# orgTestCodacy11KRepos110MB/repo-8852-ginkgo

Measured on AMD Instinct MI355X. Metric: CSR SpMV GFLOP/s (fp64, 1M-row 5-pt Poisson per GPU), higher is better.
Workload: dtype f64; 1 GPU; benchmark/spmv: CSR fp64/int32 y=Ax on 1000x1000 5-pt Poisson (n=1e6, nnz=4996000), x=sin(0.01 i); cache_state=cold: rotating over 8 copies (> 256 MiB Infinity Cache), partition=one GPU

## Files before the change

include/gkomi.h:

```cpp
#ifndef GKOMI_H_
#define GKOMI_H_

#include <stddef.h>
#include <stdint.h>

#ifdef __cplusplus
extern "C" {
#endif

typedef void* gkomi_stream_t;

enum {
    GKOMI_SUCCESS = 0,
    GKOMI_EINVAL = -1,
    GKOMI_ENOTSUPPORTED = -2,
    GKOMI_ENOTIMPL = -3,
    GKOMI_EWORKSPACE = -4,
    GKOMI_ECOMM = -5,
    GKOMI_ETRS_OVERRUN = -6
};

#define GKOMI_STATUS_CONVERGED 0x80u
#define GKOMI_STATUS_FINALIZED 0x40u
#define GKOMI_STATUS_ID_MASK 0x3fu
// ... 547 lines not shown
    gkomi_stream_t s, int64_t iterations, int64_t nnz,
    const int32_t* coo_row_idxs, const int32_t* coo_col_idxs,
    const double* coo_vals, const int32_t* l_row_ptrs,
    const int32_t* l_col_idxs, double* l_vals, const int32_t* ut_row_ptrs,
    const int32_t* ut_col_idxs, double* ut_vals);
int gkomi_factorization_initialize_row_ptrs_l_i32(
    gkomi_stream_t s, int64_t n, const int32_t* row_ptrs,
    const int32_t* col_idxs, int32_t* l_row_ptrs, void* workspace,
    size_t workspace_bytes);
int gkomi_factorization_initialize_l_f64_i32(
    gkomi_stream_t s, int64_t n, const int32_t* row_ptrs,
    const int32_t* col_idxs, const double* vals, const int32_t* l_row_ptrs,
    int32_t* l_col_idxs, double* l_vals, int diag_sqrt);
int gkomi_par_ic_init_factor_f64_i32(gkomi_stream_t s, int64_t n,
                                     const int32_t* l_row_ptrs,
                                     const int32_t* l_col_idxs, double* l_vals);
int gkomi_par_ic_compute_factor_f64_i32(gkomi_stream_t s, int64_t iterations,
                                        int64_t l_nnz,
                                        const int32_t* l_row_idxs,
                                        const double* a_lower_vals,
                                        const int32_t* l_row_ptrs,
                                        const int32_t* l_col_idxs,
                                        double* l_vals);
size_t gkomi_ilu_analysis_workspace_bytes(int64_t n);
void gkomi_ilu_tuning(int64_t* host_out);
int gkomi_ilu_analyse_i32(gkomi_stream_t s, int64_t n, const int32_t* row_ptrs,
                          const int32_t* col_idxs, void* workspace,
                          size_t workspace_bytes, int64_t* host_out);
int gkomi_ilu_compute_lu_f64_i32(gkomi_stream_t s, int64_t n,
                                 const int32_t* row_ptrs,
                                 const int32_t* col_idxs, double* vals,
                                 const void* analysis_workspace,
                                 size_t workspace_bytes);
int gkomi_ic_compute_f64_i32(gkomi_stream_t s, int64_t n,
                             const int32_t* row_ptrs, const int32_t* col_idxs,
                             double* vals, const void* analysis_workspace,
                             size_t workspace_bytes);
int gkomi_elimination_forest_host_i32(int64_t n, const int32_t* host_row_ptrs,
                                      const int32_t* host_col_idxs,
                                      int32_t* parents, int32_t* child_ptrs,
                                      int32_t* children, int32_t* postorder,
                                      int32_t* inv_postorder,
                                      int32_t* postorder_parents);
int gkomi_elimination_forest_i32(gkomi_stream_t s, int64_t n,
                                 const int32_t* row_ptrs,
                                 const int32_t* col_idxs, int32_t* parents,
                                 int32_t* child_ptrs, int32_t* children,
                                 int32_t* postorder, int32_t* inv_postorder,
                                 int32_t* postorder_parents);
size_t gkomi_cholesky_symbolic_workspace_bytes(int64_t n, int64_t nnz);
int gkomi_cholesky_symbolic_count_i32(gkomi_stream_t s, int64_t n, int64_t nnz,
                                      const int32_t* row_ptrs,
                                      const int32_t* col_idxs,
                                      const int32_t* inv_postorder,
                                      const int32_t* postorder_parents,
                                      int32_t* row_nnz, void* workspace,
                                      size_t workspace_bytes,
                                      int64_t* host_factor_nnz);
int gkomi_cholesky_symbolic_factorize_i32(
    gkomi_stream_t s, int64_t n, int64_t nnz, const int32_t* row_ptrs,
    const int32_t* col_idxs, const int32_t* postorder,
    const int32_t* inv_postorder, const int32_t* postorder_parents,
    const int32_t* out_row_ptrs, int32_t* out_cols, void* workspace,
    size_t workspace_bytes);
int gkomi_lu_initialize_f64_i32(gkomi_stream_t s, int64_t n,
                                const int32_t* a_row_ptrs,
                                const int32_t* a_col_idxs, const double* a_vals,
                                int64_t factor_nnz, const int32_t* f_row_ptrs,
                                const int32_t* f_col_idxs, double* f_vals,
                                int32_t* diag_idxs, void* workspace,
                                size_t workspace_bytes);
int gkomi_lu_factorize_f64_i32(gkomi_stream_t s, int64_t n,
                               const int32_t* f_row_ptrs,
                               const int32_t* f_col_idxs, double* f_vals,
                               const void* analysis_workspace,
                               size_t workspace_bytes);
int gkomi_lu_symbolic_supported(int has_symbolic, int symmetric_sparsity);

size_t gkomi_matrix_data_workspace_bytes(int64_t nnz);
int gkomi_matrix_data_sort_row_major_f64_i32(gkomi_stream_t s, int64_t nnz,
                                             int32_t* row_idxs,
                                             int32_t* col_idxs, double* values,
                                             void* workspace,
                                             size_t workspace_bytes);
int gkomi_matrix_data_remove_zeros_f64_i32(
    gkomi_stream_t s, int64_t nnz, const int32_t* row_idxs,
    const int32_t* col_idxs, const double* values, int32_t* out_row_idxs,
    int32_t* out_col_idxs, double* out_values, void* workspace,
    size_t workspace_bytes, int64_t* host_nnz);
int gkomi_matrix_data_sum_duplicates_f64_i32(
    gkomi_stream_t s, int64_t nnz, const int32_t* row_idxs,
    const int32_t* col_idxs, const double* values, int32_t* out_row_idxs,
    int32_t* out_col_idxs, double* out_values, void* workspace,
    size_t workspace_bytes, int64_t* host_nnz);

int gkomi_csr_sort_by_column_index_f64_i32(gkomi_stream_t s, int64_t nrows,
                                           const int32_t* row_ptrs,
                                           int32_t* col_idxs, double* vals);
int gkomi_csr_is_sorted_by_column_index_i32(gkomi_stream_t s, int64_t nrows,
                                            const int32_t* row_ptrs,
                                            const int32_t* col_idxs,
                                            void* workspace,
                                            size_t workspace_bytes,
                                            int* host_is_sorted);
size_t gkomi_csr_transpose_workspace_bytes(int64_t ncols);
int gkomi_csr_transpose_f64_i32(gkomi_stream_t s, int64_t nrows, int64_t ncols,
                                int64_t nnz, const int32_t* row_ptrs,
                                const int32_t* col_idxs, const double* vals,
                                int32_t* t_row_ptrs, int32_t* t_col_idxs,
                                double* t_vals, void* workspace,
                                size_t workspace_bytes);

size_t gkomi_csr_spgemm_workspace_bytes(int64_t a_nrows, int64_t b_ncols);
int gkomi_csr_spgemm_f64_i32(
    gkomi_stream_t s, int64_t a_nrows, int64_t a_ncols, int64_t a_nnz,
    const int32_t* a_row_ptrs, const int32_t* a_col_idxs, const double* a_vals,
    int64_t b_nrows, int64_t b_ncols, int64_t b_nnz, const int32_t* b_row_ptrs,
    const int32_t* b_col_idxs, const double* b_vals, const double* alpha,
    const double* beta, int64_t d_nrows, int64_t d_ncols, int64_t d_nnz,
    const int32_t* d_row_ptrs, const int32_t* d_col_idxs, const double* d_vals,
    int32_t* c_row_ptrs, int32_t* c_col_idxs, double* c_vals,
    int64_t* host_c_nnz, void* workspace, size_t workspace_bytes);
int gkomi_csr_spgemm_bins(int64_t out[3]);
size_t gkomi_csr_spgeam_workspace_bytes(int64_t nrows);
int gkomi_csr_spgeam_f64_i32(
    gkomi_stream_t s, int64_t nrows, int64_t ncols, const double* alpha,
    int64_t a_nnz, const int32_t* a_row_ptrs, const int32_t* a_col_idxs,
    const double* a_vals, const double* beta, int64_t b_nrows, int64_t b_ncols,
    int64_t b_nnz, const int32_t* b_row_ptrs, const int32_t* b_col_idxs,
    const double* b_vals, int32_t* c_row_ptrs, int32_t* c_col_idxs,
    double* c_vals, int64_t* host_c_nnz, void* workspace,
    size_t workspace_bytes);

typedef int (*gkomi_apply_fn)(void* ctx, gkomi_stream_t s, const double* in,
                              double* out);
size_t gkomi_cg_workspace_bytes(int64_t n, int64_t nrhs);
size_t gkomi_diag_radix_sort_workspace_bytes(int64_t n, int key_bytes, int pairs);
int gkomi_diag_radix_sort(gkomi_stream_t s, int64_t n, int key_bytes, const void* keys_in,
                          void* keys_out, const uint32_t* vals_in, uint32_t* vals_out,
                          int end_bit, void* workspace, size_t workspace_bytes);
int gkomi_diag_scan_i32(gkomi_stream_t s, int kind, const int32_t* in, int32_t* out,
                        int64_t n, void* workspace, size_t workspace_bytes);
int gkomi_diag_stream_csr_bytes(gkomi_stream_t s, int blocks, int64_t nrows,
                                int64_t nnz, const int32_t* row_ptrs,
                                const int32_t* col_idxs, const double* vals,
                                const double* b, double* c);
int gkomi_diag_poisson3d_7pt_f64_i32(gkomi_stream_t s, int64_t g, int32_t* row_ptrs,
                                     int32_t* col_idxs, double* vals);
int gkomi_diag_poisson3d_7pt_f64_i64(gkomi_stream_t s, int64_t g, int64_t* row_ptrs,
                                     int64_t* col_idxs, double* vals);
int64_t gkomi_diag_csr_evicted_applies(void);
int64_t gkomi_cg_persistent_solves(void);
int gkomi_cg_persistent_enable(int mode);
int64_t gkomi_gmres_meeting_fallbacks(void);
int gkomi_cg_solve_f64_i32(gkomi_stream_t s, int64_t n, int64_t nrhs,
                           int64_t nnz, const int32_t* row_ptrs,
                           const int32_t* col_idxs, const double* vals,
                           int spmv_strategy, int64_t max_row_nnz_hint,
                           gkomi_apply_fn precond, void* precond_ctx,
                           const double* b, double* x, int64_t max_iters,
                           double reduction_factor, int baseline, int mode,
                           int check_every, void* workspace,
                           size_t workspace_bytes, double* host_info);

int gkomi_bicgstab_initialize_f64(gkomi_stream_t s, int64_t n, int64_t nrhs,
    const double* b, int64_t b_stride, double* r, int64_t r_stride, double*
    rr, int64_t rr_stride, double* y, int64_t y_stride, double* s_vec, int64_t
    s_stride, double* t, int64_t t_stride, double* z, int64_t z_stride,
    double* v, int64_t v_stride, double* p, int64_t p_stride, double*
    prev_rho, double* rho, double* alpha, double* beta, double* gamma, double*
    omega, uint8_t* stop_status);
int gkomi_bicgstab_step_1_f64(gkomi_stream_t s, int64_t n, int64_t nrhs, const
    double* r, int64_t r_stride, double* p, int64_t p_stride, const double* v,
    int64_t v_stride, const double* rho, const double* prev_rho, const double*
    alpha, const double* omega, const uint8_t* stop_status);
int gkomi_bicgstab_step_2_f64(gkomi_stream_t s, int64_t n, int64_t nrhs, const
    double* r, int64_t r_stride, double* s_vec, int64_t s_stride, const
    double* v, int64_t v_stride, const double* rho, double* alpha, const
    double* beta, const uint8_t* stop_status);
int gkomi_bicgstab_step_3_f64(gkomi_stream_t s, int64_t n, int64_t nrhs,
    double* x, int64_t x_stride, double* r, int64_t r_stride, const double*
    s_vec, int64_t s_stride, const double* t, int64_t t_stride, const double*
    y, int64_t y_stride, const double* z, int64_t z_stride, const double*
    alpha, const double* beta, const double* gamma, double* omega, const
    uint8_t* stop_status);
int gkomi_bicgstab_finalize_f64(gkomi_stream_t s, int64_t n, int64_t nrhs,
    double* x, int64_t x_stride, const double* y, int64_t y_stride, const
    double* alpha, uint8_t* stop_status);
int gkomi_fcg_initialize_f64(gkomi_stream_t s, int64_t n, int64_t nrhs, const
    double* b, int64_t b_stride, double* r, int64_t r_stride, double* z,
    int64_t z_stride, double* p, int64_t p_stride, double* q, int64_t
    q_stride, double* t, int64_t t_stride, double* prev_rho, double* rho,
    double* rho_t, uint8_t* stop_status);
int gkomi_fcg_step_1_f64(gkomi_stream_t s, int64_t n, int64_t nrhs, double* p,
    int64_t p_stride, const double* z, int64_t z_stride, const double* rho_t,
    const double* prev_rho, const uint8_t* stop_status);
int gkomi_fcg_step_2_f64(gkomi_stream_t s, int64_t n, int64_t nrhs, double* x,
    int64_t x_stride, double* r, int64_t r_stride, double* t, int64_t
    t_stride, const double* p, int64_t p_stride, const double* q, int64_t
    q_stride, const double* beta, const double* rho, const uint8_t*
    stop_status);
int gkomi_cgs_initialize_f64(gkomi_stream_t s, int64_t n, int64_t nrhs, const
    double* b, int64_t b_stride, double* r, int64_t r_stride, double* r_tld,
    int64_t r_tld_stride, double* p, int64_t p_stride, double* q, int64_t
    q_stride, double* u, int64_t u_stride, double* u_hat, int64_t
    u_hat_stride, double* v_hat, int64_t v_hat_stride, double* t, int64_t
    t_stride, double* alpha, double* beta, double* gamma, double* prev_rho,
    double* rho, uint8_t* stop_status);
int gkomi_cgs_step_1_f64(gkomi_stream_t s, int64_t n, int64_t nrhs, const
    double* r, int64_t r_stride, double* u, int64_t u_stride, double* p,
    int64_t p_stride, const double* q, int64_t q_stride, double* beta, const
    double* rho, const double* prev_rho, const uint8_t* stop_status);
int gkomi_cgs_step_2_f64(gkomi_stream_t s, int64_t n, int64_t nrhs, const
    double* u, int64_t u_stride, const double* v_hat, int64_t v_hat_stride,
    double* q, int64_t q_stride, double* t, int64_t t_stride, double* alpha,
    const double* rho, const double* gamma, const uint8_t* stop_status);
int gkomi_cgs_step_3_f64(gkomi_stream_t s, int64_t n, int64_t nrhs, const
    double* t, int64_t t_stride, const double* u_hat, int64_t u_hat_stride,
    double* r, int64_t r_stride, double* x, int64_t x_stride, const double*
    alpha, const uint8_t* stop_status);
size_t gkomi_krylov_workspace_bytes(int64_t n, int64_t nrhs);
int gkomi_bicgstab_solve_f64_i32(gkomi_stream_t s, int64_t n, int64_t nrhs,
    int64_t nnz, const int32_t* row_ptrs, const int32_t* col_idxs, const
    double* vals, int spmv_strategy, int64_t max_row_nnz_hint, gkomi_apply_fn
    precond, void* precond_ctx, const double* b, double* x, int64_t max_iters,
    double reduction_factor, int baseline, int64_t check_every, void* workspace, size_t
    workspace_bytes, double* host_info);
int gkomi_fcg_solve_f64_i32(gkomi_stream_t s, int64_t n, int64_t nrhs, int64_t
    nnz, const int32_t* row_ptrs, const int32_t* col_idxs, const double* vals,
    int spmv_strategy, int64_t max_row_nnz_hint, gkomi_apply_fn precond, void*
    precond_ctx, const double* b, double* x, int64_t max_iters, double
    reduction_factor, int baseline, int64_t check_every, void* workspace, size_t workspace_bytes,
    double* host_info);
int gkomi_cgs_solve_f64_i32(gkomi_stream_t s, int64_t n, int64_t nrhs, int64_t
    nnz, const int32_t* row_ptrs, const int32_t* col_idxs, const double* vals,
    int spmv_strategy, int64_t max_row_nnz_hint, gkomi_apply_fn precond, void*
    precond_ctx, const double* b, double* x, int64_t max_iters, double
    reduction_factor, int baseline, int64_t check_every, void* workspace, size_t workspace_bytes,
    double* host_info);

int gkomi_bicg_initialize_f64(gkomi_stream_t s, int64_t n, int64_t nrhs, const
    double* b, int64_t b_stride, double* r, int64_t r_stride, double* z,
    int64_t z_stride, double* p, int64_t p_stride, double* q, int64_t
    q_stride, double* prev_rho, double* rho, double* r2, int64_t r2_stride,
    double* z2, int64_t z2_stride, double* p2, int64_t p2_stride, double* q2,
    int64_t q2_stride, uint8_t* stop_status);
int gkomi_bicg_step_1_f64(gkomi_stream_t s, int64_t n, int64_t nrhs, double*
    p, int64_t p_stride, const double* z, int64_t z_stride, double* p2,
    int64_t p2_stride, const double* z2, int64_t z2_stride, const double* rho,
    const double* prev_rho, const uint8_t* stop_status);
int gkomi_bicg_step_2_f64(gkomi_stream_t s, int64_t n, int64_t nrhs, double*
    x, int64_t x_stride, double* r, int64_t r_stride, double* r2, int64_t
    r2_stride, const double* p, int64_t p_stride, const double* q, int64_t
    q_stride, const double* q2, int64_t q2_stride, const double* beta, const
    double* rho, const uint8_t* stop_status);
int gkomi_ir_initialize(gkomi_stream_t s, int64_t nrhs, uint8_t* stop_status);
int gkomi_bicg_solve_f64_i32(gkomi_stream_t s, int64_t n, int64_t nrhs,
    int64_t nnz, const int32_t* row_ptrs, const int32_t* col_idxs, const
    double* vals, const int32_t* t_row_ptrs, const int32_t* t_col_idxs, const
    double* t_vals, int spmv_strategy, int64_t max_row_nnz_hint,
    gkomi_apply_fn precond, void* precond_ctx, gkomi_apply_fn precond_t, void*
    precond_t_ctx, const double* b, double* x, int64_t max_iters, double
    reduction_factor, int baseline, int64_t check_every, void* workspace,
    size_t workspace_bytes, double* host_info);
int gkomi_ir_solve_f64_i32(gkomi_stream_t s, int64_t n, int64_t nrhs, int64_t
    nnz, const int32_t* row_ptrs, const int32_t* col_idxs, const double* vals,
    int spmv_strategy, int64_t max_row_nnz_hint, gkomi_apply_fn inner, void*
    inner_ctx, double relaxation_factor, const double* b, double* x, int64_t
    max_iters, double reduction_factor, int baseline, void* workspace, size_t
    workspace_bytes, double* host_info);

int gkomi_partition_build_ranges_from_global_size(int64_t num_parts,
                                                  int64_t global_size,
                                                  int64_t* host_ranges);
int gkomi_partition_build_from_contiguous(int64_t num_parts,
                                          const int64_t* host_ranges,
                                          int64_t* host_range_bounds,
                                          int32_t* host_part_ids);
int gkomi_partition_build_from_mapping(int64_t n, const int32_t* host_mapping,
                                       int64_t* host_range_bounds,
                                       int32_t* host_part_ids,
                                       int64_t* host_num_ranges);
int gkomi_partition_build_starting_indices(const int64_t* host_range_bounds,
                                           const int32_t* host_part_ids,
                                           int64_t num_ranges,
                                           int64_t num_parts,
                                           int32_t* host_starting_indices,
                                           int32_t* host_part_sizes,
                                           int64_t* host_num_empty_parts);
int gkomi_partition_has_ordered_parts(const int32_t* host_part_ids,
                                      int64_t num_ranges, int64_t* host_result);
int gkomi_dist_vector_build_local_f64(gkomi_stream_t s, int64_t nnz,
                                      const int64_t* rows, const int64_t* cols,
                                      const double* vals, const int64_t* range_bounds,
                                      const int32_t* part_ids, const int32_t* starts,
                                      int64_t num_ranges, int32_t local_part,
                                      double* local, int64_t local_stride);
size_t gkomi_dist_build_workspace_bytes(int64_t nnz);
int gkomi_dist_build_local_nonlocal_sizes(
    gkomi_stream_t s, int64_t nnz, const int64_t* rows, const int64_t* cols,
    const int64_t* row_range_bounds, const int32_t* row_part_ids,
    const int32_t* row_starts, int64_t row_num_ranges,
    const int64_t* col_range_bounds, const int32_t* col_part_ids,
    const int32_t* col_starts, int64_t col_num_ranges, int32_t local_part,
    void* workspace, size_t workspace_bytes, int64_t host_sizes[3]);
int gkomi_dist_build_local_nonlocal_fill(
// ... 388 lines not shown
```

repo-8852-ginkgo_amd/csrc/cg_persistent.hpp:

```cpp
#pragma once
#include "cg_fused.hpp"

namespace gkomi {
namespace {

constexpr int pcg_block = 1024;
constexpr int pcg_items = 6;
constexpr int pcg_tile = pcg_block * pcg_items;
constexpr int pcg_max_rows_per_thread = 8;
constexpr int pcg_max_stride = 256;
constexpr int pcg_default_stride = 16;

struct pcg_slot {
    unsigned long long v_bits;
    unsigned long long check;
};

struct pcg_control {
    unsigned int overrun;
    unsigned int pad_[15];
    unsigned long long ticks[8];
    unsigned long long pad2_[16];
};

#ifdef GKOMI_PCG_PROFILE
#define PCG_STAMP(i)                                      \
    do {                                                  \
        const unsigned long long now_ = wall_clock64();   \
        if (blockIdx.x == 0 && threadIdx.x == 0) ctl->ticks[i] += now_ - stamp_; \
        stamp_ = now_;                                    \
    } while (0)
#else
#define PCG_STAMP(i)
#endif

typedef unsigned int pcg_u32x4 __attribute__((ext_vector_type(4)));

__device__ __forceinline__ unsigned long long pcg_key(long long meeting)
{
    return static_cast<unsigned long long>(meeting) * 0x9e3779b97f4a7c15ull;
}

__device__ __forceinline__ void pcg_publish(pcg_slot* slot, double v, long long meeting)
{
    const unsigned long long bits = static_cast<unsigned long long>(__double_as_longlong(v));
    const unsigned long long chk = bits ^ pcg_key(meeting);
    pcg_u32x4 w;
    w.x = static_cast<unsigned int>(bits);
    w.y = static_cast<unsigned int>(bits >> 32);
    w.z = static_cast<unsigned int>(chk);
    w.w = static_cast<unsigned int>(chk >> 32);
    asm volatile("global_store_dwordx4 %0, %1, off sc1" : : "v"(slot), "v"(w) : "memory");
}

__device__ __forceinline__ bool pcg_fetch(const pcg_slot* slot, long long meeting, double* v)
{
    pcg_u32x4 w;
    asm volatile("global_load_dwordx4 %0, %1, off sc1\n\ts_waitcnt vmcnt(0)" : "=v"(w) : "v"(slot) : "memory");
    const unsigned long long bits = (static_cast<unsigned long long>(w.y) << 32) | w.x;
    const unsigned long long chk = (static_cast<unsigned long long>(w.w) << 32) | w.z;
    *v = __longlong_as_double(static_cast<long long>(bits));
    return (bits ^ chk) == pcg_key(meeting);
}

constexpr int pcg_copies = 32;

__device__ __forceinline__ void pcg_sync_lds()
{
    asm volatile("s_waitcnt lgkmcnt(0)\n\ts_barrier" ::: "memory");
}

template <int Block>
__device__ __forceinline__ double pcg_block_sum(double v, double* smem)
{
    v = wave_reduce_sum(v);
    if ((threadIdx.x & 63) == 0) smem[threadIdx.x >> 6] = v;
    pcg_sync_lds();
    double total = 0.0;
#pragma unroll
    for (int w = 0; w < Block / wave_size; ++w) total += smem[w];
    pcg_sync_lds();
    return total;
}

template <int Block>
__device__ __forceinline__ bool pcg_meet(pcg_slot* slots, int stride, int nap, int nwg, long long meeting,
                                         double mine, double* smem, pcg_control* ctl, long long max_polls,
                                         double* total)
{
    constexpr int nwaves = Block / wave_size;
    pcg_slot* bank = slots + (meeting & 1) * static_cast<int64_t>(nwg + pcg_copies) * stride;
    pcg_slot* back = bank + static_cast<int64_t>(nwg) * stride;
#ifdef GKOMI_PCG_PROFILE
    const unsigned long long m0_ = wall_clock64();
#endif
    if (threadIdx.x == 0) pcg_publish(bank + blockIdx.x * stride, mine, meeting);
    bool ok = true;
    auto wait_for = [&](const pcg_slot* slot, double* v) {
        long long polls = 0;
        while (!pcg_fetch(slot, meeting, v)) {
            for (int z = 0; z < nap; ++z) __builtin_amdgcn_s_sleep(1);
            if (++polls > max_polls ||
                ((polls & 255) == 0 &&
                 __hip_atomic_load(&ctl->overrun, __ATOMIC_RELAXED, __HIP_MEMORY_SCOPE_AGENT) != 0)) {
                *v = 0.0;
                return false;
            }
        }
        return true;
    };
    if (threadIdx.x == 0) smem[nwaves] = 1.0;
    pcg_sync_lds();
    double sum = 0.0;
    if (blockIdx.x == 0) {
        double part = 0.0;
        if (static_cast<int>(threadIdx.x) < nwg) ok = wait_for(bank + threadIdx.x * stride, &part);
#ifdef GKOMI_PCG_PROFILE
        if (threadIdx.x == 0) ctl->pad2_[0] += wall_clock64() - m0_;
        if (threadIdx.x == nwg - 1) ctl->pad2_[1] += wall_clock64() - m0_;
#endif
        if (!ok) smem[nwaves] = 0.0;
        part = wave_reduce_sum(part);
        if ((threadIdx.x & 63) == 0) smem[threadIdx.x >> 6] = part;
        pcg_sync_lds();
#pragma unroll
        for (int w = 0; w < nwaves; ++w) sum += smem[w];
        ok = smem[nwaves] != 0.0;
        if (ok && threadIdx.x < pcg_copies) pcg_publish(back + threadIdx.x * stride, sum, meeting);
#ifdef GKOMI_PCG_PROFILE
        if (threadIdx.x == 0) ctl->pad2_[2] += wall_clock64() - m0_;
#endif
    } else {
        if (threadIdx.x == 0) {
            ok = wait_for(back + (blockIdx.x % pcg_copies) * stride, &sum);
#ifdef GKOMI_PCG_PROFILE
            if (blockIdx.x == 101) ctl->pad2_[3] += wall_clock64() - m0_;
            if (blockIdx.x == 101) ctl->pad2_[4] += 1;
#endif
            smem[0] = sum;
            if (!ok) smem[nwaves] = 0.0;
        }
        pcg_sync_lds();
        sum = smem[0];
        ok = smem[nwaves] != 0.0;
    }
    pcg_sync_lds();
    if (!ok) {
        if (threadIdx.x == 0) __hip_atomic_store(&ctl->overrun, 1u, __ATOMIC_RELAXED, __HIP_MEMORY_SCOPE_AGENT);
        return false;
    }
    *total = sum;
    return true;
}

template <int Block, int NV, bool Published = false, typename F>
__device__ __forceinline__ bool pcg_meet_values(pcg_slot* slots, int stride, int nap, int nwg, long long meeting,
                                                double* lsum, double* lred, double* lval, pcg_control* ctl,
                                                long long max_polls, F after_publish)
{
    static_assert(NV <= pcg_default_stride, "a workgroup's values share its slot line");
    static_assert(pcg_copies * NV <= Block, "one thread per copy and value");
    constexpr int nwaves = Block / wave_size;
    const int tid = threadIdx.x;
    pcg_slot* bank = slots + (meeting & 1) * static_cast<int64_t>(nwg + pcg_copies) * stride;
    pcg_slot* back = bank + static_cast<int64_t>(nwg) * stride;
    if (!Published && tid < NV) pcg_publish(bank + blockIdx.x * stride + tid, lsum[tid], meeting);
    after_publish();
    if (!Published) {
        if (tid == 0) lred[nwaves * NV] = 1.0;
        pcg_sync_lds();
    }
    const unsigned long long key = pcg_key(meeting);
    bool ok = true;
    if (blockIdx.x == 0) {
        if (Published) pcg_sync_lds();
        constexpr int U = 5;
        const int npairs = nwg * NV;
        for (int base = 0; base < npairs && ok; base += U * Block) {
            unsigned int pending = 0u;
#pragma unroll
            for (int u = 0; u < U; ++u) {
                if (base + u * Block + tid < npairs) pending |= 1u << u;
            }
            long long polls = 0;
            while (pending != 0u) {
                unsigned long long bits[U], chk[U];
#pragma unroll
                for (int u = 0; u < U; ++u) {
                    if ((pending >> u) & 1u) {
                        const int pr = base + u * Block + tid;
                        const pcg_slot* slot = bank + (pr / NV) * stride + pr % NV;
                        bits[u] = __hip_atomic_load(&slot->v_bits, __ATOMIC_RELAXED, __HIP_MEMORY_SCOPE_AGENT);
                        chk[u] = __hip_atomic_load(&slot->check, __ATOMIC_RELAXED, __HIP_MEMORY_SCOPE_AGENT);
                    }
                }
#pragma unroll
                for (int u = 0; u < U; ++u) {
                    if (((pending >> u) & 1u) && (bits[u] ^ chk[u]) == key) {
                        lval[base + u * Block + tid] = __longlong_as_double(static_cast<long long>(bits[u]));
                        pending &= ~(1u << u);
                    }
                }
                if (pending != 0u) {
                    for (int z = 0; z < nap; ++z) __builtin_amdgcn_s_sleep(1);
                    if (++polls > max_polls ||
                        ((polls & 255) == 0 &&
                         __hip_atomic_load(&ctl->overrun, __ATOMIC_RELAXED, __HIP_MEMORY_SCOPE_AGENT) != 0)) {
                        ok = false;
                        break;
                    }
                }
            }
        }
        if (!ok) lred[nwaves * NV] = 0.0;
        pcg_sync_lds();
        ok = lred[nwaves * NV] != 0.0;
        if (ok) {
            for (int v = tid >> 6; v < NV; v += nwaves) {
                double t = 0.0;
                for (int g = tid & 63; g < nwg; g += wave_size) t += lval[g * NV + v];
                t = wave_reduce_sum(t);
                if ((tid & 63) == 0) lsum[v] = t;
            }
        }
        pcg_sync_lds();
        ok = lred[nwaves * NV] != 0.0;
        if (ok && tid < pcg_copies * NV) pcg_publish(back + (tid / NV) * stride + tid % NV, lsum[tid % NV], meeting);
    } else {
        if (tid < NV) {
            double total = 0.0;
            long long polls = 0;
            while (!pcg_fetch(back + (blockIdx.x % pcg_copies) * stride + tid, meeting, &total)) {
                for (int z = 0; z < nap; ++z) __builtin_amdgcn_s_sleep(1);
                if (++polls > max_polls ||
                    ((polls & 255) == 0 &&
                     __hip_atomic_load(&ctl->overrun, __ATOMIC_RELAXED, __HIP_MEMORY_SCOPE_AGENT) != 0)) {
                    lred[nwaves * NV] = 0.0;
                    total = 0.0;
                    break;
                }
            }
            lsum[tid] = total;
        }
        pcg_sync_lds();
        ok = lred[nwaves * NV] != 0.0;
    }
    pcg_sync_lds();
    if (!ok) {
        if (tid == 0) __hip_atomic_store(&ctl->overrun, 1u, __ATOMIC_RELAXED, __HIP_MEMORY_SCOPE_AGENT);
        return false;
    }
    return true;
}

template <int Block>
__device__ __forceinline__ bool pcg_barrier(pcg_slot* slots, int stride, int nap, int nwg, long long meeting,
                                            double* smem, pcg_control* ctl, long long max_polls)
{
    __builtin_amdgcn_s_waitcnt(0);
    pcg_sync_lds();
    double unused;
    return pcg_meet<Block>(slots, stride, nap, nwg, meeting, 0.0, smem, ctl, max_polls, &unused);
}

template <int R, int K, int Block, bool XL = false>
__global__ __launch_bounds__(Block) void cg_persistent_kernel(
    int n, int chunk, const int32_t* __restrict__ row_ptrs, const int32_t* __restrict__ col_idxs,
    const double* __restrict__ vals, double* __restrict__ x, double* __restrict__ r, double* pbuf0,
    double* pbuf1, pcg_slot* slots, int stride, int nap, pcg_control* ctl, cg_scalars* scal,
    long long max_iters, double goal, long long max_polls, int ell_stored, int64_t ell_stride)
{
    typedef double nt_double2 __attribute__((ext_vector_type(2)));
    typedef int nt_int2 __attribute__((ext_vector_type(2)));
    constexpr int pairs = pcg_items / 2;
    __shared__ __attribute__((aligned(16))) double prod[K > 0 ? 2 : (Block * pcg_items)];
    __shared__ unsigned int lcol[K > 0 ? K * R * Block : 1];
    __shared__ double lx[XL ? R * Block : 1];
    __shared__ double smem[Block / wave_size + 1];
    const int nwg = gridDim.x;
    const int tid = threadIdx.x;
    const int b0 = min(static_cast<int>(blockIdx.x) * chunk, n);
    const int b1 = min(b0 + chunk, n);
    const bool ell = K > 0 && ell_stored > 0;
    const int nz0 = ell ? 0 : row_ptrs[b0];
    const int nz1 = ell ? 0 : row_ptrs[b1];
    const int nnz_total = ell ? 0 : row_ptrs[n];
    int ra[R], rb[R];
    double xr[XL ? 1 : R], rr[R], pr[R], qr[R];
#pragma unroll
    for (int k = 0; k < R; ++k) {
        const int row = b0 + k * Block + tid;
        ra[k] = rb[k] = nz1;
        rr[k] = 0.0;
        if (XL) {
            lx[k * Block + tid] = 0.0;
        } else {
            xr[k] = 0.0;
        }
        pr[k] = 0.0;
        if (row < b1) {
            if (!ell) {
                ra[k] = row_ptrs[row];
                rb[k] = row_ptrs[row + 1];
            }
            if (XL) {
                lx[k * Block + tid] = x[row];
            } else {
                xr[k] = x[row];
            }
            rr[k] = r[row];
        }
    }
    constexpr int KK = K > 0 ? K : 1;
    double mv[R][KK];
    unsigned int present[R];
    if (K > 0) {
        bool fits = n <= (1 << 28) && (!ell || ell_stored <= K);
#pragma unroll
        for (int k = 0; k < R; ++k) {
            const int row = b0 + k * Block + tid;
            const int len = rb[k] - ra[k];
            fits &= ell || len <= K;
            present[k] = 0;
#pragma unroll
            for (int e = 0; e < KK; ++e) {
                bool have = false;
                double val = 0.0;
                int col = 0;
                if (ell) {
                    if (row < b1 && e < ell_stored) {
                        col = col_idxs[row + e * ell_stride];
                        val = vals[row + e * ell_stride];
                        have = col != -1;
                    }
                } else if (e < len) {
                    col = col_idxs[ra[k] + e];
                    val = vals[ra[k] + e];
                    have = true;
                }
                mv[k][e] = have ? val : 0.0;
                present[k] |= have ? (1u << e) : 0u;
                lcol[(e * R + k) * Block + tid] = have ? static_cast<unsigned int>(col) * 8u : 0u;
            }
        }
        double misfits = 0.0;
        const double mine = pcg_block_sum<Block>(fits ? 0.0 : 1.0, smem);
        if (!pcg_meet<Block>(slots, stride, nap, gridDim.x, 1, mine, smem, ctl, max_polls, &misfits)) return;
        if (misfits != 0.0) {
            if (blockIdx.x == 0 && tid == 0) {
                __hip_atomic_store(&ctl->overrun, 2u, __ATOMIC_RELAXED, __HIP_MEMORY_SCOPE_AGENT);
            }
            return;
        }
    }
    const double orig = scal->orig_tau;
    double prev = scal->rho[1];
    long long meeting = K > 0 ? 1 : 0;
    long long it = 0;
    uint8_t st = 0;
    double rho = 0.0, tau = 0.0;
    bool broken = false;
#ifdef GKOMI_PCG_PROFILE
    unsigned long long stamp_ = wall_clock64();
#endif
    while (true) {
        if (tid >= Block - wave_size) asm volatile("buffer_inv sc1" ::: "memory");
        double acc = 0.0;
#pragma unroll
        for (int k = 0; k < R; ++k) acc += rr[k] * rr[k];
        const double mine = pcg_block_sum<Block>(acc, smem);
        if (!pcg_meet<Block>(slots, stride, nap, nwg, ++meeting, mine, smem, ctl, max_polls, &rho)) {
            broken = true;
            break;
        }
        PCG_STAMP(0);
        tau = sqrt(rho);
        if (it >= max_iters) {
            st = id_iteration | GKOMI_STATUS_FINALIZED;
        } else if (tau < goal * orig) {
            st = GKOMI_STATUS_CONVERGED | id_residual | GKOMI_STATUS_FINALIZED;
        }
        if (st) break;
        const bool restart = prev == 0.0;
        const double factor = restart ? 0.0 : rho / prev;
        double* pbuf = (it & 1) ? pbuf1 : pbuf0;
#pragma unroll
        for (int k = 0; k < R; ++k) {
            const int row = b0 + k * Block + tid;
            pr[k] = restart ? rr[k] : rr[k] + factor * pr[k];
            if (row < b1) __hip_atomic_store(pbuf + row, pr[k], __ATOMIC_RELAXED, __HIP_MEMORY_SCOPE_AGENT);
        }
        if (!pcg_barrier<Block>(slots, stride, nap, nwg, ++meeting, smem, ctl, max_polls)) {
            broken = true;
            break;
        }
        PCG_STAMP(1);
        PCG_STAMP(2);
#pragma unroll
        for (int k = 0; k < R; ++k) qr[k] = 0.0;
        if (K > 0) {
            constexpr int G = R >= 2 ? 2 : 1;
#pragma unroll
            for (int k0 = 0; k0 < R; k0 += G) {
                double pv[G][KK];
#pragma unroll
                for (int g = 0; g < G; ++g) {
#pragma unroll
                    for (int e = 0; e < KK; ++e) {
                        const unsigned int off = lcol[(e * R + k0 + g) * Block + tid];
                        pv[g][e] = *reinterpret_cast<const double*>(reinterpret_cast<const char*>(pbuf) + off);
                    }
                }
#pragma unroll
                for (int g = 0; g < G; ++g) {
                    double acc_row = 0.0;
#pragma unroll
                    for (int e = 0; e < KK; ++e) {
                        acc_row = (present[k0 + g] >> e) & 1u ? acc_row + mv[k0 + g][e] * pv[g][e] : acc_row;
                    }
                    qr[k0 + g] = acc_row;
                }
            }
        } else {
            for (int t0 = nz0 & ~1; t0 < nz1; t0 += (Block * pcg_items)) {
                double2 v[pairs];
                int2 ci[pairs];
    #pragma unroll
                for (int u = 0; u < pairs; ++u) {
                    const int k = t0 + 2 * (tid + u * Block);
                    v[u] = make_double2(0.0, 0.0);
                    ci[u] = make_int2(0, 0);
                    if (k < nz1) {
                        if (k + 1 < nnz_total) {
                            const nt_double2 tv =
                                __builtin_nontemporal_load(reinterpret_cast<const nt_double2*>(vals + k));
                            const nt_int2 tc =
                                __builtin_nontemporal_load(reinterpret_cast<const nt_int2*>(col_idxs + k));
                            v[u] = make_double2(tv.x, tv.y);
                            ci[u] = make_int2(tc.x, tc.y);
                        } else {
                            v[u].x = vals[k];
                            ci[u].x = col_idxs[k];
                        }
                    }
                }
                double2 pv[pairs];
    #pragma unroll
                for (int u = 0; u < pairs; ++u) {
                    pv[u].x = pbuf[ci[u].x];
                    pv[u].y = pbuf[ci[u].y];
                }
    #pragma unroll
                for (int u = 0; u < pairs; ++u) {
                    *reinterpret_cast<double2*>(prod + 2 * (tid + u * Block)) =
                        make_double2(v[u].x * pv[u].x, v[u].y * pv[u].y);
                }
                __syncthreads();
                const int t1 = t0 + (Block * pcg_items);
    #pragma unroll
                for (int k = 0; k < R; ++k) {
                    const int lo = max(ra[k], t0), hi = min(rb[k], t1);
                    for (int j = lo; j < hi; ++j) qr[k] += prod[j - t0];
                }
                __syncthreads();
            }
        }
        PCG_STAMP(3);
        acc = 0.0;
#pragma unroll
        for (int k = 0; k < R; ++k) acc += pr[k] * qr[k];
        const double mine_pq = pcg_block_sum<Block>(acc, smem);
        double pq = 0.0;
        if (!pcg_meet<Block>(slots, stride, nap, nwg, ++meeting, mine_pq, smem, ctl, max_polls, &pq)) {
            broken = true;
            break;
        }
        PCG_STAMP(4);
        if (pq != 0.0) {
            const double alpha = rho / pq;
#pragma unroll
            for (int k = 0; k < R; ++k) {
                if (XL) {
                    lx[k * Block + tid] += alpha * pr[k];
                } else {
                    xr[k] += alpha * pr[k];
                }
                rr[k] -= alpha * qr[k];
            }
        }
        prev = rho;
        ++it;
        PCG_STAMP(5);
    }
#pragma unroll
    for (int k = 0; k < R; ++k) {
        const int row = b0 + k * Block + tid;
        if (row < b1) {
            x[row] = XL ? lx[k * Block + tid] : xr[k];
            r[row] = rr[k];
        }
    }
    if (blockIdx.x == 0 && tid == 0 && !broken) {
        scal->rho[it & 1] = rho;
        scal->rho[(it + 1) & 1] = prev;
        scal->tau = tau;
        scal->stop_iter = it;
        scal->status = st;
    }
}

__global__ void pcg_clear_kernel(pcg_slot* slots, int stride, int count, pcg_control* ctl)
{
    for (int i = threadIdx.x; i < count; i += blockDim.x) {
        slots[static_cast<int64_t>(i) * stride].v_bits = 0;
        slots[static_cast<int64_t>(i) * stride].check = 0;
    }
    if (threadIdx.x == 0) ctl->overrun = 0;
    if (threadIdx.x < 8) ctl->ticks[threadIdx.x] = 0;
    if (threadIdx.x < 16) ctl->pad2_[threadIdx.x] = 0;
}

}
}
```

repo-8852-ginkgo_amd/csrc/cg_solver.hip:

```cpp
#include "cg_persistent.hpp"
#include "krylov_driver.hpp"

#include <atomic>
#include <cstdio>
#include <cstdlib>

namespace gkomi {
namespace {

struct cg_layout {
    solver_layout base;
    size_t pcg_ctl, pcg_slots, total;
};

cg_layout make_cg_layout(int64_t n, int64_t nrhs)
{
    cg_layout l{};
    l.base = make_solver_layout(n, nrhs, 4);
    auto align256 = [](size_t bytes) { return (bytes + 255) / 256 * 256; };
    l.pcg_ctl = l.base.total;
    l.pcg_slots = l.pcg_ctl + align256(sizeof(pcg_control));
    l.total = l.pcg_slots + align256(sizeof(pcg_slot) * 2 * (max_parts + pcg_copies) * pcg_max_stride);
    return l;
}

std::atomic<int64_t> pcg_solves{0};
std::atomic<int> pcg_mode{[] {
    const char* e = std::getenv("GKOMI_CG_PERSISTENT");
    return e == nullptr ? 1 : std::atoi(e);
}()};

}
}

using namespace gkomi;

extern "C" int64_t gkomi_cg_persistent_solves(void) { return pcg_solves.load(); }
extern "C" int gkomi_cg_persistent_enable(int mode)
{
    if (mode < 0 || mode > 2) return GKOMI_EINVAL;
    pcg_mode.store(mode);
    return GKOMI_SUCCESS;
}

extern "C" size_t gkomi_cg_workspace_bytes(int64_t n, int64_t nrhs)
{
    if (n < 0 || nrhs <= 0) return 0;
    return make_cg_layout(n, nrhs).total;
}

namespace {
#define PCG_TRY(expr)                        \
    do {                                     \
        const int err_ = (expr);             \
        if (err_) return -(1000 + err_);     \
    } while (0)
int persistent_cg(const driver_common& c, const solve_request& req, const spmv_dot_plan& spmv, double* r, double* p,
                  double* q, cg_scalars* scal, void* ctl_mem, void* slot_mem, cg_scalars* result)
{
    const gkomi_stream_t s = c.s;
    hipStream_t stream = c.stream;
    const int64_t n = c.n;
    const sysmat& A = c.A;
    double* x = req.x;
    cg_scalars polled{};
    const int persistent_mode = pcg_mode.load();
    static const int cus = device_cu_count();
    const int64_t pcg_chunk = cus > 0 ? ceildiv(n, cus) : 0;
    const gkomi_ell_ctx* ell = !A.is_csr() && A.op == &gkomi_ell_matrix_apply_cb && A.ctx != nullptr
                                   ? static_cast<const gkomi_ell_ctx*>(A.ctx)
                                   : nullptr;
    if (ell != nullptr && (ell->nrows != n || ell->ncols != n || ell->stride < n)) ell = nullptr;
    const int64_t pcg_hint = ell != nullptr ? ell->num_stored_per_row
                                            : spmv.A.hint;
    const bool pcg_fits_matrix =
        pcg_hint >= 1 && pcg_hint <= 7 && ceildiv(pcg_chunk, 512) <= 8;
    const bool pcg_fits_vectors = ceildiv(pcg_chunk, pcg_block) <= pcg_max_rows_per_thread;
    if (persistent_mode >= 1 && c.precond == nullptr && (spmv.csr || ell != nullptr) && cus >= 8 &&
        cus <= max_parts &&
        n >= 64 * static_cast<int64_t>(cus) &&
        (pcg_fits_matrix || (persistent_mode >= 2 && pcg_fits_vectors && ell == nullptr)) &&
        persistent_try_acquire()) {
        struct release_guard {
            ~release_guard() { persistent_release(); }
        } release;
        const sysmat& M = spmv.A;
        const int32_t* m_row_ptrs = ell != nullptr ? nullptr : M.row_ptrs;
        const int32_t* m_col_idxs = ell != nullptr ? ell->col_idxs : M.col_idxs;
        const double* m_vals = ell != nullptr ? ell->vals : M.vals;
        const int ell_stored = ell != nullptr ? static_cast<int>(ell->num_stored_per_row) : 0;
        const int64_t ell_stride = ell != nullptr ? ell->stride : 0;
        pcg_control* ctl = static_cast<pcg_control*>(ctl_mem);
        pcg_slot* slots = static_cast<pcg_slot*>(slot_mem);
        const int chunk = static_cast<int>(ceildiv(n, cus));
        const int rows_per_thread = static_cast<int>(ceildiv(chunk, pcg_block));
        const long long max_polls = [] {
            const char* e = std::getenv("GKOMI_MEET_MAX_POLLS");
            return e != nullptr && e[0] != 0 ? std::max(1ll, atoll(e)) : 1ll << 22;
        }();
        static const int stride = [] {
            const char* e = std::getenv("GKOMI_PCG_STRIDE");
            const int v = e != nullptr ? std::atoi(e) : pcg_default_stride;
            return v >= 1 && v <= pcg_max_stride ? v : pcg_default_stride;
        }();
        static const bool resident_on = [] {
            const char* e = std::getenv("GKOMI_PCG_RESIDENT");
            return e == nullptr || e[0] != '0';
        }();
        static const int nap = [] {
            const char* e = std::getenv("GKOMI_PCG_NAP");
            const int v = e != nullptr ? std::atoi(e) : 1;
            return v >= 0 && v <= 64 ? v : 1;
        }();
        hipLaunchKernelGGL(pcg_clear_kernel, dim3(1), dim3(256), 0, stream, slots, stride, 2 * (cus + pcg_copies), ctl);
#define GKOMI_PCG(R, KR, BLOCK)                                                                        \
hipLaunchKernelGGL((cg_persistent_kernel<R, KR, BLOCK, (KR == 7 && R == 8)>), dim3(cus), dim3(BLOCK), 0, stream, \
                   static_cast<int>(n), chunk, m_row_ptrs, m_col_idxs, m_vals, x, r, p, q, slots,  \
                   stride, nap, ctl, scal, static_cast<long long>(c.max_iters), c.reduction,       \
                   max_polls, ell_stored, ell_stride)
        const int rows_per_thread_512 = static_cast<int>(ceildiv(chunk, 512));
        const bool resident = pcg_fits_matrix && resident_on;
        if (resident && pcg_hint <= 5) {
            if (rows_per_thread_512 <= 2) {
                GKOMI_PCG(2, 5, 512);
            } else if (rows_per_thread_512 <= 4) {
                GKOMI_PCG(4, 5, 512);
            } else {
                GKOMI_PCG(8, 5, 512);
            }
        } else if (resident) {
            if (rows_per_thread_512 <= 2) {
                GKOMI_PCG(2, 7, 512);
            } else if (rows_per_thread_512 <= 4) {
                GKOMI_PCG(4, 7, 512);
            } else {
                GKOMI_PCG(8, 7, 512);
            }
        } else if (rows_per_thread <= 1) {
            GKOMI_PCG(1, 0, 1024);
        } else if (rows_per_thread <= 2) {
            GKOMI_PCG(2, 0, 1024);
        } else if (rows_per_thread <= 4) {
            GKOMI_PCG(4, 0, 1024);
        } else {
            GKOMI_PCG(8, 0, 1024);
        }
#undef GKOMI_PCG
        PCG_TRY(check_launch());
        pcg_control hctl{};
        PCG_TRY(static_cast<int>(hipMemcpyAsync(&hctl, ctl, sizeof(pcg_control), hipMemcpyDeviceToHost, stream)));
        PCG_TRY(static_cast<int>(hipMemcpyAsync(&polled, scal, sizeof(cg_scalars), hipMemcpyDeviceToHost, stream)));
        PCG_TRY(static_cast<int>(hipStreamSynchronize(stream)));
#ifdef GKOMI_PCG_PROFILE
        fprintf(stderr, "pcg phases (us per iteration, workgroup 0): meet rho %.2f | p + barrier %.2f | inv %.2f | "
                        "spmv %.2f | meet pq %.2f | update %.2f over %lld iterations\n",
                hctl.ticks[0] * 0.01 / (polled.stop_iter + 1), hctl.ticks[1] * 0.01 / (polled.stop_iter + 1),
                hctl.ticks[2] * 0.01 / (polled.stop_iter + 1), hctl.ticks[3] * 0.01 / (polled.stop_iter + 1),
                hctl.ticks[4] * 0.01 / (polled.stop_iter + 1), hctl.ticks[5] * 0.01 / (polled.stop_iter + 1),
                polled.stop_iter);
        fprintf(stderr, "pcg meeting (us, mean over %llu meetings): own slot seen %.2f | last slot seen %.2f | total "
                        "published %.2f | workgroup 101 has the total %.2f\n",
                hctl.pad2_[4], hctl.pad2_[0] * 0.01 / hctl.pad2_[4], hctl.pad2_[1] * 0.01 / hctl.pad2_[4],
                hctl.pad2_[2] * 0.01 / hctl.pad2_[4], hctl.pad2_[3] * 0.01 / hctl.pad2_[4]);
#endif
        if (hctl.overrun == 0 && (polled.status & GKOMI_STATUS_ID_MASK)) {
            pcg_solves.fetch_add(1);
            *result = polled;
            return 1;
        } else {
            PCG_TRY(gkomi_dense_copy_f64(s, n, 1, req.b, 1, r, 1));
            PCG_TRY(A.apply(s, 1, c.neg_one, x, c.one, r));
            PCG_TRY(gkomi_dense_fill_f64(s, n, 1, p, 1, 0.0));
            hipLaunchKernelGGL(cg_init_scalars_kernel, dim3(1), dim3(1), 0, stream, scal, c.orig_tau,
                               req.baseline == 2 ? 1 : 0);
        }
    }
    return 0;
}
#undef PCG_TRY

int cg_solve_impl(const solve_request& req, int mode)
{
    const gkomi_stream_t s = req.s;
    const int64_t n = req.n, nrhs = req.nrhs;
    if (mode == 1 && n == 0) mode = 0;
    bool reference = false;
    const int too_many_rows = fused_preflight(req, &reference);
    if (mode == 1 && nrhs == 1 && (reference || reinterpret_cast<uintptr_t>(req.workspace) % 16 != 0)) mode = 0;
    if (n < 0 || nrhs <= 0 || req.max_iters < 0) return GKOMI_EINVAL;
    if (req.baseline < 0 || req.baseline > 2 || (mode != 0 && mode != 1)) return GKOMI_EINVAL;
    if (mode == 1 && nrhs != 1) return GKOMI_ENOTSUPPORTED;
    GKOMI_TRY(too_many_rows);
    const cg_layout l = make_cg_layout(n, nrhs);
    driver_common c;
    GKOMI_TRY(c.init(req, 6, l.base, l.total));
    c.iteration_id = id_iteration;
    c.residual_id = id_residual;
    hipStream_t stream = c.stream;
    const sysmat& A = c.A;
    double *x = req.x, *r = c.vec(0), *z = c.vec(1), *p = c.vec(2), *q = c.vec(3);
    double *prev_rho = c.scalars, *rho = prev_rho + nrhs, *beta = rho + nrhs;
    GKOMI_TRY(gkomi_cg_initialize_f64(s, n, nrhs, req.b, nrhs, r, nrhs, z, nrhs, p,
                                      nrhs, q, nrhs, prev_rho, rho, c.stop_status));
    GKOMI_TRY(c.start(req, r));

    if (mode == 0) {
        c.check_every = 1;
        int64_t iter = -1;
        while (true) {
            GKOMI_TRY(c.apply_precond(r, z));
            GKOMI_TRY(c.dot(r, z, rho));
            ++iter;
            bool stop = false;
            GKOMI_TRY(c.check(iter, r, true, 1, &stop));
            if (stop) break;
            GKOMI_TRY(gkomi_cg_step_1_f64(s, n, nrhs, p, nrhs, z, nrhs, rho, prev_rho, c.stop_status));
            GKOMI_TRY(c.spmv(p, q));
            GKOMI_TRY(c.dot(p, q, beta));
            GKOMI_TRY(gkomi_cg_step_2_f64(s, n, nrhs, x, nrhs, r, nrhs, p, nrhs, q, nrhs, beta, rho,
                                          c.stop_status));
            std::swap(prev_rho, rho);
        }
        return c.finish(c.stop_iter(), r, req.host_info);
    } else {
        fused_driver<cg_scalars> f(c);
        cg_scalars* scal = f.scal;
        double *part_a = f.spmv_partials(), *part_b = f.spmv_partials(), *part_c = f.spmv_partials();
        const int g = f.g, nb = f.nb;
        const spmv_dot_plan& spmv = f.spmv;
        const gkomi_apply_fn precond = c.precond;
        hipLaunchKernelGGL(cg_init_scalars_kernel, dim3(1), dim3(1), 0, stream, scal, c.orig_tau,
                           req.baseline == 2 ? 1 : 0);
        GKOMI_TRY(check_launch());
        {
            cg_scalars polled{};
            const int done = persistent_cg(c, req, spmv, r, p, q, scal, c.ws + l.pcg_ctl, c.ws + l.pcg_slots, &polled);
            if (done < 0) return -done - 1000;
            if (done == 1) {
                fill_host_info(req.host_info, polled.stop_iter, polled.status, polled.tau, polled.orig_tau);
                return precond_status(precond, c.precond_ctx, s);
            }
        }
        const double* zz = precond == nullptr ? r : z;
        const gkomi_jacobi_ctx* jac =
            precond == &gkomi_jacobi_apply_cb ? static_cast<const gkomi_jacobi_ctx*>(c.precond_ctx) : nullptr;
        int ng = g;
        auto precondition = [&](bool first) -> int {
            if (jac != nullptr) {
                const int got = jacobi_apply_dot_launch(s, jac, r, z, part_a, part_b, spmv_dot_partials_room(n),
                                                        &scal->status);
                if (got < 0) return -got - 1000;
                if (got > 0) {
                    ng = got;
                    return 0;
                }
                jac = nullptr;
            }
            GKOMI_TRY(c.apply_precond(r, z));
            hipLaunchKernelGGL(cg_dot2_partials_kernel, dim3(g), dim3(fblock), 0, stream, n, r, z,
                               first ? static_cast<const cg_scalars*>(nullptr) : static_cast<const cg_scalars*>(scal),
                               part_a, first ? part_b : static_cast<double*>(nullptr));
            return check_launch();
        };
        if (precond != nullptr) {
            GKOMI_TRY(precondition(true));
        } else {
            hipLaunchKernelGGL(cg_dot2_partials_kernel, dim3(g), dim3(fblock), 0, stream, n, r, zz,
                               static_cast<const cg_scalars*>(nullptr), part_a, static_cast<double*>(nullptr));
            GKOMI_TRY(check_launch());
        }
        const double* tau_part = precond == nullptr ? part_a : part_b;
        host_watch& watch = f.watch;
        auto issue = [&](long long i, bool) -> int {
            hipLaunchKernelGGL(cg_fused_step1_kernel, dim3(g), dim3(fblock), 0, stream, n, p, zz,
                               part_a, ng, tau_part, jac != nullptr ? ng : g, scal, i,
                               static_cast<long long>(c.max_iters), c.reduction, watch.dev);
            if (spmv.fused()) {
                GKOMI_TRY(spmv.launch(stream, p, q, part_c, &scal->status));
            } else {
                GKOMI_TRY(A.apply(s, 1, nullptr, p, nullptr, q));
                hipLaunchKernelGGL(cg_dot2_partials_kernel, dim3(g), dim3(fblock), 0, stream, n, p, q,
                                   static_cast<const cg_scalars*>(scal), part_c,
                                   static_cast<double*>(nullptr));
            }
            hipLaunchKernelGGL(cg_fused_step2_kernel, dim3(g), dim3(fblock), 0, stream, n, x, r, p,
                               q, part_c, nb, scal, i, precond == nullptr ? part_a : part_b);
            if (precond != nullptr) GKOMI_TRY(precondition(false));
            return check_launch();
        };
        return f.solve(issue, req.host_info);
    }
}
}

extern "C" int gkomi_cg_solve_f64_i32(
    gkomi_stream_t s, int64_t n, int64_t nrhs, int64_t nnz,
    const int32_t* row_ptrs, const int32_t* col_idxs, const double* vals,
    int spmv_strategy, int64_t max_row_nnz_hint, gkomi_apply_fn precond,
    void* precond_ctx, const double* b, double* x, int64_t max_iters,
    double reduction_factor, int baseline, int mode, int check_every,
    void* workspace, size_t workspace_bytes, double* host_info)
{
    return cg_solve_impl({s, n, nrhs, make_csr_sysmat(n, nnz, row_ptrs, col_idxs, vals, spmv_strategy, max_row_nnz_hint),
        precond, precond_ctx, b, x, max_iters, reduction_factor, baseline, check_every, workspace, workspace_bytes,
        host_info}, mode);
}

extern "C" int gkomi_cg_solve_fused_op_f64(gkomi_stream_t s, int64_t n, gkomi_matrix_apply_fn matrix,
                                           void* matrix_ctx, gkomi_apply_fn precond, void* precond_ctx,
                                           const double* b, double* x, int64_t max_iters,
                                           double reduction_factor, int baseline, int64_t check_every,
                                           void* workspace, size_t workspace_bytes, double* host_info)
{
    if (matrix == nullptr) return GKOMI_EINVAL;
    return cg_solve_impl({s, n, 1, make_op_sysmat(n, matrix, matrix_ctx),
        precond, precond_ctx, b, x, max_iters, reduction_factor, baseline, std::min<int64_t>(check_every, 1 << 20),
        workspace, workspace_bytes, host_info}, 1);
}

// ... 12 lines not shown
```

Baseline: 615.2 GFLOP/s.

## Replace global barrier with neighbour hand-off in persistent CG kernel

In the persistent CG kernel with a resident matrix, each workgroup now computes the column window its rows touch and, if that window spans at most one wave of workgroups, publishes its p-ready flag and waits only on the owning neighbour workgroups instead of a grid-wide barrier. The cache invalidate is skipped in that mode. The XL local-x variant is also enabled for K=5. This targets CG solves, not the SpMV benchmark being measured, so the SpMV metric should be largely unaffected. It adds risk around memory visibility when the global invalidate is skipped.

```diff
diff --git a/include/gkomi.h b/include/gkomi.h
--- a/include/gkomi.h
+++ b/include/gkomi.h
@@ -723,6 +723,8 @@
 int64_t gkomi_diag_csr_evicted_applies(void);
 int64_t gkomi_cg_persistent_solves(void);
 int gkomi_cg_persistent_enable(int mode);
+int gkomi_cg_persistent_handoff(int mode);
+int64_t gkomi_cg_persistent_handoff_solves(void);
 int64_t gkomi_gmres_meeting_fallbacks(void);
 int gkomi_cg_solve_f64_i32(gkomi_stream_t s, int64_t n, int64_t nrhs,
                            int64_t nnz, const int32_t* row_ptrs,
diff --git a/repo-8852-ginkgo_amd/csrc/cg_persistent.hpp b/repo-8852-ginkgo_amd/csrc/cg_persistent.hpp
--- a/repo-8852-ginkgo_amd/csrc/cg_persistent.hpp
+++ b/repo-8852-ginkgo_amd/csrc/cg_persistent.hpp
@@ -18,7 +18,8 @@
 
 struct pcg_control {
     unsigned int overrun;
-    unsigned int pad_[15];
+    unsigned int handoff;
+    unsigned int pad_[14];
     unsigned long long ticks[8];
     unsigned long long pad2_[16];
 };
@@ -263,12 +264,59 @@
     return pcg_meet<Block>(slots, stride, nap, nwg, meeting, 0.0, smem, ctl, max_polls, &unused);
 }
 
+__device__ __forceinline__ void pcg_handoff_publish(pcg_slot* slots, int stride, int nwg, long long meeting)
+{
+    asm volatile("s_waitcnt vmcnt(0)" ::: "memory");
+    pcg_sync_lds();
+    pcg_slot* bank = slots + (meeting & 1) * static_cast<int64_t>(nwg + pcg_copies) * stride;
+    if (threadIdx.x == 0) pcg_publish(bank + blockIdx.x * stride, 0.0, meeting);
+}
+
+template <int Block>
+__device__ __forceinline__ bool pcg_handoff_wait(const pcg_slot* slots, int stride, int nap, int nwg,
+                                                 long long meeting, int wlo, int width, double* smem,
+                                                 pcg_control* ctl, long long max_polls)
+{
+    constexpr int nwaves = Block / wave_size;
+    const pcg_slot* bank = slots + (meeting & 1) * static_cast<int64_t>(nwg + pcg_copies) * stride;
+    if (threadIdx.x < wave_size) {
+        int lane = threadIdx.x;
+        asm volatile("" : "+v"(lane));
+        bool have = lane >= width;
+        bool ok = true;
+        long long polls = 0;
+        while (true) {
+            if (!have) {
+                double unused;
+                have = pcg_fetch(bank + static_cast<int64_t>(wlo + lane) * stride, meeting, &unused);
+            }
+            if (__all(have)) break;
+            for (int z = 0; z < nap; ++z) __builtin_amdgcn_s_sleep(1);
+            if (++polls > max_polls ||
+                ((polls & 255) == 0 &&
+                 __hip_atomic_load(&ctl->overrun, __ATOMIC_RELAXED, __HIP_MEMORY_SCOPE_AGENT) != 0)) {
+                ok = false;
+                break;
+            }
+        }
+        if (ok) {
+            __builtin_amdgcn_fence(__ATOMIC_ACQUIRE, "agent");
+            asm volatile("s_waitcnt vmcnt(0)" ::: "memory");
+        }
+        if (threadIdx.x == 0) smem[nwaves] = ok ? 1.0 : 0.0;
+    }
+    pcg_sync_lds();
+    const bool ok = smem[nwaves] != 0.0;
+    if (!ok && threadIdx.x == 0) __hip_atomic_store(&ctl->overrun, 1u, __ATOMIC_RELAXED, __HIP_MEMORY_SCOPE_AGENT);
+    return ok;
+}
+
 template <int R, int K, int Block, bool XL = false>
 __global__ __launch_bounds__(Block) void cg_persistent_kernel(
     int n, int chunk, const int32_t* __restrict__ row_ptrs, const int32_t* __restrict__ col_idxs,
     const double* __restrict__ vals, double* __restrict__ x, double* __restrict__ r, double* pbuf0,
     double* pbuf1, pcg_slot* slots, int stride, int nap, pcg_control* ctl, cg_scalars* scal,
-    long long max_iters, double goal, long long max_polls, int ell_stored, int64_t ell_stride)
+    long long max_iters, double goal, long long max_polls, int ell_stored, int64_t ell_stride, int handoff_on)
 {
     typedef double nt_double2 __attribute__((ext_vector_type(2)));
     typedef int nt_int2 __attribute__((ext_vector_type(2)));
@@ -276,6 +324,7 @@
     __shared__ __attribute__((aligned(16))) double prod[K > 0 ? 2 : (Block * pcg_items)];
     __shared__ unsigned int lcol[K > 0 ? K * R * Block : 1];
     __shared__ double lx[XL ? R * Block : 1];
+    __shared__ int lwin[2];
     __shared__ double smem[Block / wave_size + 1];
     const int nwg = gridDim.x;
     const int tid = threadIdx.x;
@@ -314,8 +363,15 @@
     constexpr int KK = K > 0 ? K : 1;
     double mv[R][KK];
     unsigned int present[R];
+    bool handoff = false;
+    int wlo = 0, width = 0;
     if (K > 0) {
         bool fits = n <= (1 << 28) && (!ell || ell_stored <= K);
+        int cmin = n, cmax = -1;
+        if (tid == 0) {
+            lwin[0] = n;
+            lwin[1] = -1;
+        }
 #pragma unroll
         for (int k = 0; k < R; ++k) {
             const int row = b0 + k * Block + tid;
@@ -341,17 +397,39 @@
                 mv[k][e] = have ? val : 0.0;
                 present[k] |= have ? (1u << e) : 0u;
                 lcol[(e * R + k) * Block + tid] = have ? static_cast<unsigned int>(col) * 8u : 0u;
-            }
-        }
+                cmin = have ? min(cmin, col) : cmin;
+                cmax = have ? max(cmax, col) : cmax;
+            }
+        }
+        pcg_sync_lds();
+        if (cmax >= 0) {
+            atomicMin(&lwin[0], cmin);
+            atomicMax(&lwin[1], cmax);
+        }
+        constexpr double wide_unit = 1048576.0;
         double misfits = 0.0;
-        const double mine = pcg_block_sum<Block>(fits ? 0.0 : 1.0, smem);
+        double mine = pcg_block_sum<Block>(fits ? 0.0 : 1.0, smem);
+        const int wmin = lwin[0], wmax = lwin[1];
+        bool wide = false;
+        if (wmax >= 0) {
+            wide = wmin < 0 || wmax >= n;
+            wlo = wide ? 0 : wmin / chunk;
+            width = wide ? 0 : wmax / chunk - wlo + 1;
+            wide |= width > wave_size;
+        }
+        wlo = __builtin_amdgcn_readfirstlane(wlo);
+        width = __builtin_amdgcn_readfirstlane(width);
+        mine += wide ? wide_unit : 0.0;
         if (!pcg_meet<Block>(slots, stride, nap, gridDim.x, 1, mine, smem, ctl, max_polls, &misfits)) return;
+        handoff = handoff_on != 0 && misfits < wide_unit;
+        if (misfits >= wide_unit) misfits -= wide_unit * floor(misfits / wide_unit);
         if (misfits != 0.0) {
             if (blockIdx.x == 0 && tid == 0) {
                 __hip_atomic_store(&ctl->overrun, 2u, __ATOMIC_RELAXED, __HIP_MEMORY_SCOPE_AGENT);
             }
             return;
         }
+        if (handoff && blockIdx.x == 0 && tid == 0) ctl->handoff = 1u;
     }
     const double orig = scal->orig_tau;
     double prev = scal->rho[1];
@@ -364,7 +442,7 @@
     unsigned long long stamp_ = wall_clock64();
 #endif
     while (true) {
-        if (tid >= Block - wave_size) asm volatile("buffer_inv sc1" ::: "memory");
+        if (!handoff && tid >= Block - wave_size) asm volatile("buffer_inv sc1" ::: "memory");
         double acc = 0.0;
 #pragma unroll
         for (int k = 0; k < R; ++k) acc += rr[k] * rr[k];
@@ -390,14 +468,23 @@
             pr[k] = restart ? rr[k] : rr[k] + factor * pr[k];
             if (row < b1) __hip_atomic_store(pbuf + row, pr[k], __ATOMIC_RELAXED, __HIP_MEMORY_SCOPE_AGENT);
         }
-        if (!pcg_barrier<Block>(slots, stride, nap, nwg, ++meeting, smem, ctl, max_polls)) {
-            broken = true;
-            break;
-        }
-        PCG_STAMP(1);
-        PCG_STAMP(2);
 #pragma unroll
         for (int k = 0; k < R; ++k) qr[k] = 0.0;
+        if (K > 0 && handoff) {
+            pcg_handoff_publish(slots, stride, nwg, ++meeting);
+            PCG_STAMP(1);
+            if (!pcg_handoff_wait<Block>(slots, stride, nap, nwg, meeting, wlo, width, smem, ctl, max_polls)) {
+                broken = true;
+                break;
+            }
+            PCG_STAMP(2);
+        } else {
+            if (!pcg_barrier<Block>(slots, stride, nap, nwg, ++meeting, smem, ctl, max_polls)) {
+                broken = true;
+                break;
+            }
+            PCG_STAMP(1);
+        }
         if (K > 0) {
             constexpr int G = R >= 2 ? 2 : 1;
 #pragma unroll
@@ -516,6 +603,7 @@
         slots[static_cast<int64_t>(i) * stride].check = 0;
     }
     if (threadIdx.x == 0) ctl->overrun = 0;
+    if (threadIdx.x == 0) ctl->handoff = 0;
     if (threadIdx.x < 8) ctl->ticks[threadIdx.x] = 0;
     if (threadIdx.x < 16) ctl->pad2_[threadIdx.x] = 0;
 }
diff --git a/repo-8852-ginkgo_amd/csrc/cg_solver.hip b/repo-8852-ginkgo_amd/csrc/cg_solver.hip
--- a/repo-8852-ginkgo_amd/csrc/cg_solver.hip
+++ b/repo-8852-ginkgo_amd/csrc/cg_solver.hip
@@ -29,6 +29,11 @@
     const char* e = std::getenv("GKOMI_CG_PERSISTENT");
     return e == nullptr ? 1 : std::atoi(e);
 }()};
+std::atomic<int64_t> pcg_handoff_solves{0};
+std::atomic<int> pcg_handoff{[] {
+    const char* e = std::getenv("GKOMI_PCG_HANDOFF");
+    return e == nullptr || std::atoi(e) != 0 ? 1 : 0;
+}()};
 
 }
 }
@@ -40,6 +45,14 @@
 {
     if (mode < 0 || mode > 2) return GKOMI_EINVAL;
     pcg_mode.store(mode);
+    return GKOMI_SUCCESS;
+}
+
+extern "C" int64_t gkomi_cg_persistent_handoff_solves(void) { return pcg_handoff_solves.load(); }
+extern "C" int gkomi_cg_persistent_handoff(int mode)
+{
+    if (mode < 0 || mode > 1) return GKOMI_EINVAL;
+    pcg_handoff.store(mode);
     return GKOMI_SUCCESS;
 }
 
@@ -112,12 +125,13 @@
             const int v = e != nullptr ? std::atoi(e) : 1;
             return v >= 0 && v <= 64 ? v : 1;
         }();
+        const int handoff_on = pcg_handoff.load();
         hipLaunchKernelGGL(pcg_clear_kernel, dim3(1), dim3(256), 0, stream, slots, stride, 2 * (cus + pcg_copies), ctl);
 #define GKOMI_PCG(R, KR, BLOCK)                                                                        \
-hipLaunchKernelGGL((cg_persistent_kernel<R, KR, BLOCK, (KR == 7 && R == 8)>), dim3(cus), dim3(BLOCK), 0, stream, \
+hipLaunchKernelGGL((cg_persistent_kernel<R, KR, BLOCK, (KR > 0 && R == 8)>), dim3(cus), dim3(BLOCK), 0, stream, \
                    static_cast<int>(n), chunk, m_row_ptrs, m_col_idxs, m_vals, x, r, p, q, slots,  \
                    stride, nap, ctl, scal, static_cast<long long>(c.max_iters), c.reduction,       \
-                   max_polls, ell_stored, ell_stride)
+                   max_polls, ell_stored, ell_stride, handoff_on)
         const int rows_per_thread_512 = static_cast<int>(ceildiv(chunk, 512));
         const bool resident = pcg_fits_matrix && resident_on;
         if (resident && pcg_hint <= 5) {
@@ -152,12 +166,12 @@
         PCG_TRY(static_cast<int>(hipMemcpyAsync(&polled, scal, sizeof(cg_scalars), hipMemcpyDeviceToHost, stream)));
         PCG_TRY(static_cast<int>(hipStreamSynchronize(stream)));
 #ifdef GKOMI_PCG_PROFILE
-        fprintf(stderr, "pcg phases (us per iteration, workgroup 0): meet rho %.2f | p + barrier %.2f | inv %.2f | "
-                        "spmv %.2f | meet pq %.2f | update %.2f over %lld iterations\n",
-                hctl.ticks[0] * 0.01 / (polled.stop_iter + 1), hctl.ticks[1] * 0.01 / (polled.stop_iter + 1),
-                hctl.ticks[2] * 0.01 / (polled.stop_iter + 1), hctl.ticks[3] * 0.01 / (polled.stop_iter + 1),
-                hctl.ticks[4] * 0.01 / (polled.stop_iter + 1), hctl.ticks[5] * 0.01 / (polled.stop_iter + 1),
-                polled.stop_iter);
+        fprintf(stderr, "pcg phases (us per iteration, workgroup 0, hand-off %u): meet rho %.2f | p + publish %.2f | "
+                        "wait + acquire %.2f | spmv %.2f | meet pq %.2f | update %.2f over %lld iterations\n",
+                hctl.handoff, hctl.ticks[0] * 0.01 / (polled.stop_iter + 1),
+                hctl.ticks[1] * 0.01 / (polled.stop_iter + 1), hctl.ticks[2] * 0.01 / (polled.stop_iter + 1),
+                hctl.ticks[3] * 0.01 / (polled.stop_iter + 1), hctl.ticks[4] * 0.01 / (polled.stop_iter + 1),
+                hctl.ticks[5] * 0.01 / (polled.stop_iter + 1), polled.stop_iter);
         fprintf(stderr, "pcg meeting (us, mean over %llu meetings): own slot seen %.2f | last slot seen %.2f | total "
                         "published %.2f | workgroup 101 has the total %.2f\n",
                 hctl.pad2_[4], hctl.pad2_[0] * 0.01 / hctl.pad2_[4], hctl.pad2_[1] * 0.01 / hctl.pad2_[4],
@@ -165,6 +179,7 @@
 #endif
         if (hctl.overrun == 0 && (polled.status & GKOMI_STATUS_ID_MASK)) {
             pcg_solves.fetch_add(1);
+            if (hctl.handoff != 0) pcg_handoff_solves.fetch_add(1);
             *result = polled;
             return 1;
         } else {
```

Result: no change. 612.4 GFLOP/s (-0.5%).
